# cschin/Peregrine

Hardware: AMD Instinct MI355X
Metric: confirmed overlaps/sec (ovlp_t records, index+overlap stages, seqdb resident in HBM) (higher is better)
Workload: dtype u8/u32 integer

## Files before the change

peregrine_amd/csrc/pgx_align.hip:

```cpp

#include "pgx_internal.h"

namespace pgx {
namespace {

__device__ __forceinline__ uint64_t load_u64_unaligned(const uint8_t *p) {
  uint64_t v;
  __builtin_memcpy(&v, p, 8);
  return v;
}
struct U128 {
  uint64_t lo, hi;
};
__device__ __forceinline__ U128 load_u128_unaligned(const uint8_t *p) {
  U128 v;
  __builtin_memcpy(&v, p, 16);
  return v;
}
__device__ __forceinline__ int match8(uint64_t qa, uint64_t ta, int qs, int ts) {
  const uint64_t diff = ((qa >> qs) ^ (ta >> ts)) & 0x0F0F0F0F0F0F0F0FULL;
  return diff ? (__builtin_ctzll(diff) >> 3) : 8;
}
__device__ __forceinline__ uint64_t ballot64(bool p) { return __builtin_amdgcn_ballot_w64(p); }
template <int CTRL>
__device__ __forceinline__ int dpp_max(int v) {
  return max(v, __builtin_amdgcn_update_dpp(0, v, CTRL, 0xf, 0xf, true));
}
template <int GL>
__device__ __forceinline__ int group_max_i32(int v) {
  static_assert(GL == 4 || GL == 8, "a group is a quad or half a DPP row");
  v = dpp_max<0xB1>(v);
  v = dpp_max<0x4E>(v);
  return GL == 8 ? dpp_max<0x141>(v) : v;
}
template <int GL>
__device__ __forceinline__ uint32_t group_bits(uint64_t wave_mask, int gbase) {
  return (uint32_t)(wave_mask >> gbase) & ((1u << GL) - 1u);
}
template <int CTRL>
__device__ __forceinline__ int dpp_min(int v) {
  return min(v, __builtin_amdgcn_update_dpp(0, v, CTRL, 0xf, 0xf, true));
}
template <int GL>
__device__ __forceinline__ int group_min_i32(int v) {
  v = dpp_min<0xB1>(v);
  v = dpp_min<0x4E>(v);
  return GL == 8 ? dpp_min<0x141>(v) : v;
}
__device__ __forceinline__ uint32_t ffbl_or_ones(uint32_t v) {
  uint32_t r;
  asm("v_ffbl_b32 %0, %1" : "=v"(r) : "v"(v));
  return r;
}
__device__ __forceinline__ int group_lane(int v, int gb4, int l) { return __builtin_amdgcn_ds_bpermute(gb4 + (l << 2), v); }

template <int CTRL, int ROW_MASK>
__device__ __forceinline__ int dpp_max_step(int v) {
  return max(v, __builtin_amdgcn_update_dpp(v, v, CTRL, ROW_MASK, 0xf, false));
}
__device__ __forceinline__ int wave_max_i32(int v) {
  v = dpp_max_step<0x111, 0xf>(v);
  v = dpp_max_step<0x112, 0xf>(v);
  v = dpp_max_step<0x114, 0xf>(v);
  v = dpp_max_step<0x118, 0xf>(v);
  v = dpp_max_step<0x142, 0xa>(v);
  v = dpp_max_step<0x143, 0xc>(v);
  return __builtin_amdgcn_readlane(v, 63);
}


}

__device__ __forceinline__ int match16p(const uint8_t *q, uint32_t xq, const uint8_t *t, uint32_t yt) {
  uint2 qd, td;
  __builtin_memcpy(&qd, q + (xq >> 4) * 4, 8), __builtin_memcpy(&td, t + (yt >> 4) * 4, 8);
  const uint32_t df = __builtin_amdgcn_alignbit(qd.y, qd.x, (xq & 15) << 1) ^ __builtin_amdgcn_alignbit(td.y, td.x, (yt & 15) << 1);
  return (int)min(ffbl_or_ones(df) >> 1, 16u);
}
__device__ __forceinline__ uint32_t target_offset(const pgx_align_key &) { return 0u; }
__device__ __forceinline__ uint32_t target_offset(const pgx_align_key2 &k) { return k.t_off; }
template <bool PACKED, typename KEY = pgx_align_key>
__device__ __forceinline__ void align_one_per_wave(const uint8_t *__restrict__ seq, const uint64_t *__restrict__ roff,
                                                   const uint32_t *__restrict__ rlen, const KEY *__restrict__ keys, uint32_t a, int band,
                                                   int ring, pgx_match *__restrict__ out) {
  static_assert(!PACKED || std::is_same_v<KEY, pgx_align_key>, "a target offset is honoured by the byte form only");
  extern __shared__ int32_t V[];
  constexpr int PB = PACKED ? 16 : 8;
  const int lane = threadIdx.x;
  const KEY key = keys[a];
  const uint32_t len0 = rlen[key.rid0], len1 = rlen[key.rid1];
  const uint8_t *q = PACKED ? seq + (roff[key.rid0] + (key.dir0 ? (len0 + 15u) >> 4 : 0u) + (key.q_off >> 4)) * 4 : seq + roff[key.rid0] + key.q_off;
  const uint8_t *t = PACKED ? seq + (roff[key.rid1] + (key.dir1 ? (len1 + 15u) >> 4 : 0u)) * 4 : seq + roff[key.rid1] + target_offset(key);
  const uint32_t qo = PACKED ? key.q_off & 15u : 0u;
  const int q_len = (int)(len0 - key.q_off);
  const int t_len = (int)(len1 - target_offset(key));
  const int qs = key.dir0 ? 4 : 0, ts = key.dir1 ? 4 : 0;
  const int max_d = (int)(0.3 * (double)(q_len + t_len));
  const int band_size = band * 2;
  const int mask = ring - 1;
  for (int i = lane; i < ring; i += 64) V[i] = 0;
  __syncthreads();

  int best_m = -1, min_k = 0, max_k = 0;
  uint32_t longest = 0;
  bool started = false, matched = false;
  int q_bgn = 0, t_bgn = 0, q_m_end = 0, t_m_end = 0, q_end = 0, t_end = 0, dist = 0;

  for (int d = 0; d < max_d; ++d) {
    if (max_k - min_k > band_size) break;
    const int nk = max_k >= min_k ? ((max_k - min_k) >> 1) + 1 : 0;
    int x = 0, y = 0;
    for (int base = 0; base < nk && !matched; base += 64) {
      const int j = base + lane;
      const bool active = j < nk;
      const int k = min_k + 2 * j;
      int x1 = 0, y1 = 0;
      x = 0, y = 0;
      bool more = false;
      if (active) {
        const int va = V[(k - 1) & mask], vb = V[(k + 1) & mask];
        x = (k == min_k || (k != max_k && va < vb)) ? vb : va + 1;
        y = x - k;
        x1 = x, y1 = y;
        const int rem = min(q_len - x, t_len - y);
        if (rem > 0) {
          int m = PACKED ? match16p(q, qo + (uint32_t)x, t, (uint32_t)y) : match8(load_u64_unaligned(q + x), load_u64_unaligned(t + y), qs, ts);
          m = min(m, rem);
          x += m, y += m;
          more = (m == PB) && (rem > PB);
        }
      }
      uint64_t mm = ballot64(more);
      while (mm) {
        const int L = __builtin_ctzll(mm);
        const int xs = __builtin_amdgcn_readlane(x, L), ys = __builtin_amdgcn_readlane(y, L);
        const int rem = min(q_len - xs, t_len - ys);
        const int off = lane * PB;
        int m = 0;
        if (off < rem)
          m = min(PACKED ? match16p(q, qo + (uint32_t)(xs + off), t, (uint32_t)(ys + off))
                         : match8(load_u64_unaligned(q + xs + off), load_u64_unaligned(t + ys + off), qs, ts), rem - off);
        const uint64_t stop = ballot64(m < PB);
        int ext;
        if (stop) {
          const int f = __builtin_ctzll(stop);
          ext = PB * f + __builtin_amdgcn_readlane(m, f);
        } else {
          ext = 64 * PB;
        }
        if (lane == L) x += ext, y += ext;
        if (stop || ext >= rem) mm &= mm - 1;
      }
      const int ext = x - x1;
      const bool hit = active && (x >= q_len || y >= t_len);
      const uint64_t hitmask = ballot64(hit);
      const int hl = hitmask ? __builtin_ctzll(hitmask) : 64;
      const bool valid = active && lane <= hl;
      if (!started) {
        const uint64_t m = ballot64(valid && ext > 16);
        if (m) {
          const int l = __builtin_ctzll(m);
          q_bgn = __builtin_amdgcn_readlane(x1, l), t_bgn = __builtin_amdgcn_readlane(y1, l);
          started = true;
        }
      }
      if (ballot64(valid && (uint32_t)ext > longest)) {
        const int mx = wave_max_i32(valid ? ext : -1);
        const int l = __builtin_ctzll(ballot64(valid && ext == mx));
        longest = (uint32_t)mx;
        q_m_end = __builtin_amdgcn_readlane(x, l), t_m_end = __builtin_amdgcn_readlane(y, l);
      }
      if (valid) V[k & mask] = x;
      best_m = max(best_m, wave_max_i32(valid ? x + y : -1));
      if (hitmask) {
        matched = true;
        q_end = __builtin_amdgcn_readlane(x, hl), t_end = __builtin_amdgcn_readlane(y, hl);
      }
    }
    __syncthreads();
    if (matched) {
      dist = d;
      break;
    }
    int new_min = max_k, new_max = min_k;
    const int thr = best_m - band;
    for (int base = 0; base < nk; base += 64) {
      const int j = base + lane;
      const int k2 = min_k + 2 * j;
      int u;
      if (nk <= 64) u = x + y;
      else u = j < nk ? 2 * V[k2 & mask] - k2 : 0;
      const uint64_t m = ballot64(j < nk && u >= thr);
      if (m) {
        new_min = min(new_min, min_k + 2 * (base + __builtin_ctzll(m)));
        new_max = max(new_max, min_k + 2 * (base + 63 - __builtin_clzll(m)));
      }
    }
    max_k = new_max + 1;
    min_k = new_min - 1;
  }
  if (lane == 0) {
    pgx_match r;
    if (matched) {
      r.q_bgn = q_bgn, r.t_bgn = t_bgn, r.q_end = q_end, r.t_end = t_end, r.dist = dist;
      r.m_size = (q_end - q_bgn + t_end - t_bgn + 2 * dist) / 2;
    } else {
      r.q_bgn = 0, r.t_bgn = 0, r.q_end = 0, r.t_end = 0, r.dist = 0, r.m_size = 0;
    }
    r.q_m_end = q_m_end, r.t_m_end = t_m_end;
    out[a] = r;
  }
}
template <bool PACKED>
__global__ __launch_bounds__(64) void k_align1(const uint8_t *__restrict__ seq, const uint64_t *__restrict__ roff,
                                              const uint32_t *__restrict__ rlen,
                                              const pgx_align_key *__restrict__ keys, uint32_t n, int band,
                                              int ring, pgx_match *__restrict__ out) {
  if (blockIdx.x < n) align_one_per_wave<PACKED>(seq, roff, rlen, keys, blockIdx.x, band, ring, out);
}
__global__ __launch_bounds__(64) void k_align1t(const uint8_t *__restrict__ seq, const uint64_t *__restrict__ roff, const uint32_t *__restrict__ rlen,
                                               const pgx_align_key2 *__restrict__ keys, uint32_t n, int band, int ring, pgx_match *__restrict__ out) {
  if (blockIdx.x < n) align_one_per_wave<false, pgx_align_key2>(seq, roff, rlen, keys, blockIdx.x, band, ring, out);
}
__global__ __launch_bounds__(64) void k_align1_handon(const uint8_t *__restrict__ seq, const uint64_t *__restrict__ roff,
                                                     const uint32_t *__restrict__ rlen, const pgx_align_key *__restrict__ keys, uint32_t n, int band,
                                                     int ring, pgx_match *__restrict__ out, const uint32_t *__restrict__ nflag,
                                                     uint32_t *__restrict__ hand_n, uint32_t *__restrict__ hand_list) {
  if (blockIdx.x >= n) return;
  const pgx_align_key key = keys[blockIdx.x];
  if ((nflag[key.rid0] | nflag[key.rid1]) & 1u) {
    if (threadIdx.x == 0) hand_list[atomicAdd(hand_n, 1u)] = blockIdx.x;
    return;
  }
  align_one_per_wave<true>(seq, roff, rlen, keys, blockIdx.x, band, ring, out);
}
template <bool PACKED>
__global__ __launch_bounds__(64) void k_align1_list(const uint8_t *__restrict__ seq, const uint64_t *__restrict__ roff,
                                                   const uint32_t *__restrict__ rlen, const pgx_align_key *__restrict__ keys,
                                                   const uint32_t *__restrict__ list_n, const uint32_t *__restrict__ list, int band, int ring,
                                                   pgx_match *__restrict__ out) {
  const uint32_t cnt = *list_n;
  for (uint32_t i = blockIdx.x; i < cnt; i += gridDim.x) {
    __syncthreads();
    align_one_per_wave<PACKED>(seq, roff, rlen, keys, list[i], band, ring, out);
  }
}


enum { PH_FETCH = 0, PH_STEP = 1, PH_ROUND = 2, PH_SNAKE = 3, PH_END = 4, PH_BAND = 5, PH_DONE = 6 };
#define PH_SYNC() __builtin_amdgcn_fence(__ATOMIC_RELEASE, "wavefront"), __builtin_amdgcn_fence(__ATOMIC_ACQUIRE, "wavefront")
template <typename VT, bool PACKED, int GL>
__global__ __launch_bounds__(1024, 8) void k_align_ph(const uint8_t *__restrict__ seq, const uint64_t *__restrict__ roff,
                                                      const uint32_t *__restrict__ rlen, const pgx_align_key *__restrict__ keys,
                                                      uint32_t n, int band, int ring, pgx_match *__restrict__ out,
                                                      uint32_t *__restrict__ counter, const uint32_t *__restrict__ redo_n,
                                                      const uint32_t *__restrict__ redo_list, uint32_t *__restrict__ esc_n,
                                                      uint32_t *__restrict__ esc_list, const uint32_t *__restrict__ nflag, uint32_t seg,
                                                      uint32_t iter_limit) {
  extern __shared__ int32_t Vall[];
  __shared__ unsigned long long s_state;
  __shared__ uint32_t s_lock;
  const int lane = threadIdx.x & 63, gl = lane & (GL - 1), gbase = lane & ~(GL - 1), gb4 = gbase << 2;
  VT *V = reinterpret_cast<VT *>(Vall) + ((threadIdx.x >> 6) * (64 / GL) + lane / GL) * ring;
  if (threadIdx.x == 0) s_state = (unsigned long long)seg, s_lock = 0u;
  __syncthreads();
  const int mask2 = (ring - 1) << 1, band_size = band * 2;
  const auto slot = [&](int kd) -> VT & {
    return *reinterpret_cast<VT *>(reinterpret_cast<char *>(V) + (kd & mask2) * (int)(sizeof(VT) / 2));
  };
  constexpr int SL = PACKED ? 32 : 16;
  constexpr int PROBE = PACKED ? 16 : 8;
  if (redo_list) n = *redo_n;
  const uint32_t iter_budget = esc_list && iter_limit ? iter_limit : 0xFFFFFFFFu;
  uint32_t qo = 0, to = 0;
  uint32_t iters = 0;
  uint32_t c_next = 0, c_end = 0;

  int phase = PH_FETCH;
  uint32_t a = 0;
  const uint8_t *q = seq, *t = seq;
  int q_len = 0, t_len = 0, qs = 0, ts = 0, max_d = 0, d = 0;
  int best_m = -1, min_k = 0, max_k = 0, nk = 0, base = 0, bbase = 0, new_min = 0, new_max = 0;
  uint32_t longest = 0;
  bool started = false;
  int q_bgn = 0, t_bgn = 0, q_m_end = 0, t_m_end = 0;
  int x = 0, y = 0, x1 = 0, y1 = 0, k = 0;
  bool active = false;
  uint32_t gm = 0;

#ifdef PGX_ALIGN_STATS
  uint32_t my_iters = 0;
  int my_maxnk = 0;
  bool has_cand = false;
  const bool stats_on = !redo_list || redo_n == esc_n + 3;
#endif
  for (;;) {
#ifdef PGX_ALIGN_STATS
    if (phase == PH_FETCH && has_cand && gl == 0 && stats_on) {
      const uint32_t b = my_iters ? 31u - (uint32_t)__builtin_clz(my_iters) : 0u;
      atomicAdd(counter + 1 + min(b, 31u), 1u);
#ifdef PGX_ALIGN_STATS_NK
      atomicAdd(counter + 33 + min((uint32_t)my_maxnk, 31u), 1u);
#else
      atomicAdd(counter + 33 + min(b, 31u), my_iters);
#endif
    }
    if (phase == PH_FETCH) has_cand = false, my_iters = 0, my_maxnk = 0;
    my_maxnk = max(my_maxnk, phase == PH_ROUND || phase == PH_STEP ? nk : 0);
    ++my_iters;
#endif
    ++iters;
    constexpr uint32_t RETRY = 0xFFFFFFFFu;
    const bool fetching = phase == PH_FETCH;
    const uint64_t fw = ballot64(fetching);
    uint32_t na = 0;
    if (fw) {
      constexpr uint32_t CHUNK = 64 / GL;
      const uint64_t need = fw & (GL == 8 ? 0x0101010101010101ULL : 0x1111111111111111ULL);
      const uint32_t cnt = (uint32_t)__builtin_popcountll(need);
      const uint32_t r = __builtin_amdgcn_mbcnt_hi((uint32_t)(need >> 32), __builtin_amdgcn_mbcnt_lo((uint32_t)need, 0u));
      const uint32_t avail = __builtin_amdgcn_readfirstlane(c_end - c_next);
      na = c_next + r;
      if (avail < cnt) {
        uint32_t got = RETRY;
        if (lane == 0) {
          unsigned long long o = atomicAdd(&s_state, (unsigned long long)CHUNK);
          if ((uint32_t)o < seg) {
            got = (uint32_t)(o >> 32) + (uint32_t)o;
          } else if (atomicCAS(&s_lock, 0u, 1u) == 0u) {
            o = atomicAdd(&s_state, (unsigned long long)CHUNK);
            if ((uint32_t)o < seg) {
              got = (uint32_t)(o >> 32) + (uint32_t)o;
            } else {
              got = atomicAdd(counter, seg);
              atomicExch(&s_state, ((unsigned long long)got << 32) | CHUNK);
            }
            atomicExch(&s_lock, 0u);
          }
        }
        got = __builtin_amdgcn_readfirstlane(got);
        if (got == RETRY) {
          if (r >= avail) na = RETRY;
          c_next = c_end = 0;
        } else {
          if (r >= avail) na = got + (r - avail);
          c_next = got + (cnt - avail), c_end = got + CHUNK;
        }
      } else {
        c_next += cnt;
      }
    }
    if (fetching) {
      iters = 0;
      na = (uint32_t)group_lane((int)na, gb4, 0);
      if (na == RETRY) {
      } else if (na >= n) {
        phase = PH_DONE;
      } else {
#ifdef PGX_ALIGN_STATS
        has_cand = true;
#endif
        a = redo_list ? redo_list[na] : na;
        const pgx_align_key key = keys[a];
        const uint32_t len0 = rlen[key.rid0], len1 = rlen[key.rid1];
        if (PACKED) {
          q = seq + (roff[key.rid0] + (key.dir0 ? (len0 + 15u) >> 4 : 0u) + (key.q_off >> 4)) * 4;
          t = seq + (roff[key.rid1] + (key.dir1 ? (len1 + 15u) >> 4 : 0u)) * 4;
          qo = key.q_off & 15u, to = 0;
        } else {
          q = seq + roff[key.rid0] + key.q_off;
          t = seq + roff[key.rid1];
        }
        q_len = (int)(len0 - key.q_off);
        t_len = (int)len1;
        qs = key.dir0 ? 4 : 0, ts = key.dir1 ? 4 : 0;
        max_d = (int)(0.3 * (double)(q_len + t_len));
        d = 0, best_m = -1, min_k = 0, max_k = 0, longest = 0;
        started = false;
        q_bgn = t_bgn = q_m_end = t_m_end = 0;
        if (gl == 0) slot(2) = (VT)0;
        phase = PH_STEP;
        if (PACKED && ((nflag[key.rid0] | nflag[key.rid1]) & 1u)) {
          if (gl == 0) esc_list[n + atomicAdd(esc_n + 1, 1u)] = a;
          phase = PH_FETCH;
        }
      }
    }
    if (!ballot64(phase != PH_DONE)) break;
    PH_SYNC();

    if (iters > iter_budget && phase == PH_STEP && !(d >= max_d || max_k - min_k > band_size)) {
      if (gl == 0) esc_list[atomicAdd(esc_n, 1u)] = a;
      phase = PH_FETCH;
    }
    if (phase == PH_STEP) {
      const int width = max_k - min_k;
      if (d >= max_d || width > band_size) {
        if (gl == 0) {
          pgx_match r;
          r.m_size = 0, r.dist = 0, r.q_bgn = 0, r.q_end = 0, r.t_bgn = 0, r.t_end = 0;
          r.t_m_end = t_m_end, r.q_m_end = q_m_end;
          out[a] = r;
        }
        phase = PH_FETCH;
      } else if (width < 0) {
        nk = 0, base = 0, bbase = 0, new_min = max_k, new_max = min_k, phase = PH_BAND;
      } else {
        nk = (width >> 1) + 1, base = 0, phase = PH_ROUND;
      }
    }

    int probe_full = 0;
    if (phase == PH_ROUND) {
      const int j = base + gl;
      active = j < nk;
      k = min_k + 2 * j;
      if (active) {
        const int va = (int)slot(k - d), vb = (int)slot(k - d + 2);
        x = (k == min_k || (k != max_k && va < vb)) ? vb : va + 1;
        y = x - k;
        x1 = x, y1 = y;
        const int rem = min(q_len - x, t_len - y);
        if (rem > 0) {
          int m;
          if (PACKED) {
            const uint32_t xq = qo + (uint32_t)x, yt = to + (uint32_t)y;
            uint2 qd, td;
            __builtin_memcpy(&qd, q + (xq >> 4) * 4, 8), __builtin_memcpy(&td, t + (yt >> 4) * 4, 8);
            const uint32_t df = __builtin_amdgcn_alignbit(qd.y, qd.x, (xq & 15) << 1) ^ __builtin_amdgcn_alignbit(td.y, td.x, (yt & 15) << 1);
            m = (int)min(ffbl_or_ones(df) >> 1, 16u);
          } else {
            m = match8(load_u64_unaligned(q + x), load_u64_unaligned(t + y), qs, ts);
          }
          probe_full = (int)min((uint32_t)m, (uint32_t)(rem - 1));
          m = (int)min((uint32_t)m, (uint32_t)rem);
          x += m, y += m;
        }
      }
    }
    {
      asm volatile("" : "+v"(probe_full));
      const uint32_t g = group_bits<GL>(ballot64(probe_full >= PROBE), gbase);
      if (phase == PH_ROUND) gm = g, phase = g ? PH_SNAKE : PH_END;
    }

    {
      const bool sn = phase == PH_SNAKE;
      if (ballot64(sn)) {
        const int L = __builtin_ctz(gm | (1u << GL));
        const int xs = group_lane(x, gb4, L), ys = group_lane(y, gb4, L);
        const int rem = min(q_len - xs, t_len - ys);
        const int off = gl * SL;
        int e = GL * SL;
        if (sn) {
          e = off;
          if (off < rem) {
            int m;
            if (PACKED) {
              const uint32_t xq = qo + (uint32_t)(xs + off), yt = to + (uint32_t)(ys + off);
              uint4 qd, td;
              __builtin_memcpy(&qd, q + (xq >> 4) * 4, 16), __builtin_memcpy(&td, t + (yt >> 4) * 4, 16);
              const uint32_t qsh = (xq & 15) << 1, tsh = (yt & 15) << 1;
              const uint32_t d0 = __builtin_amdgcn_alignbit(qd.y, qd.x, qsh) ^ __builtin_amdgcn_alignbit(td.y, td.x, tsh);
              const uint32_t d1 = __builtin_amdgcn_alignbit(qd.z, qd.y, qsh) ^ __builtin_amdgcn_alignbit(td.z, td.y, tsh);
              m = (int)min(min(ffbl_or_ones(d0), ffbl_or_ones(d1) | 32u) >> 1, 32u);
            } else {
              const U128 qa = load_u128_unaligned(q + xs + off), ta = load_u128_unaligned(t + ys + off);
              m = match8(qa.lo, ta.lo, qs, ts);
              if (m == 8) m += match8(qa.hi, ta.hi, qs, ts);
            }
            m = (int)min((uint32_t)m, (uint32_t)(rem - off));
            e = m < SL ? off + m : GL * SL;
          }
        }
        const int ext = group_min_i32<GL>(e);
        if (sn) {
          if (gl == L) x += ext, y += ext;
          if (ext < GL * SL || ext >= rem) gm &= gm - 1;
          if (!gm) phase = PH_END;
        }
      }
    }

    {
      const bool e = phase == PH_END;
      const int ext = x - x1;
      const bool hit = e && active && (x >= q_len || y >= t_len);
      const uint64_t hitw = ballot64(hit);
      int hl = GL;
      uint32_t hitm = 0;
      if (hitw) {
        hitm = group_bits<GL>(hitw, gbase);
        if (hitm) hl = __builtin_ctz(hitm);
        asm volatile("" : "+v"(hl));
      }
      const bool valid = e && active && gl <= hl;
      {
        const uint64_t sw = ballot64((valid && !started ? ext : 0) > 16);
        if (sw) {
          const uint32_t m = group_bits<GL>(sw, gbase);
          const int l = m ? __builtin_ctz(m) : 0;
          const int bx = group_lane(x1, gb4, l), by = group_lane(y1, gb4, l);
          if (m) q_bgn = bx, t_bgn = by, started = true;
        }
      }
      const int ev = valid ? ext : -1;
      if (ballot64(ev > (int)longest)) {
        const int mx = group_max_i32<GL>(ev);
        const uint32_t m = group_bits<GL>(ballot64(valid && ext == mx), gbase);
        const int l = m ? __builtin_ctz(m) : 0;
        const int ex = group_lane(x, gb4, l), ey = group_lane(y, gb4, l);
        if (e && mx >= 0 && (uint32_t)mx > longest) longest = (uint32_t)mx, q_m_end = ex, t_m_end = ey;
      }
      if (valid) slot(k - d) = (VT)x;
      const int u = x + y;
      {
        const int s = group_max_i32<GL>(valid ? u : -1);
        if (e) best_m = max(best_m, s);
      }
      bool matched = false;
      if (hitw) {
        const int ex = group_lane(x, gb4, hl & (GL - 1)), ey = group_lane(y, gb4, hl & (GL - 1));
        if (e && hitm) {
          matched = true;
          if (gl == 0) {
            pgx_match r;
            r.q_bgn = q_bgn, r.t_bgn = t_bgn, r.q_end = ex, r.t_end = ey, r.dist = d;
            r.m_size = (ex - q_bgn + ey - t_bgn + 2 * d) / 2;
            r.t_m_end = t_m_end, r.q_m_end = q_m_end;
            out[a] = r;
          }
        }
      }
      const uint32_t qm = group_bits<GL>(ballot64((e && active ? u : INT32_MIN) >= best_m - band), gbase);
      const bool wide_step = e && !matched && nk > GL;
      if (ballot64(wide_step)) {
        const bool last = wide_step && base + GL >= nk;
        if (wide_step) {
          if (base == 0) new_min = max_k, new_max = min_k;
          if (qm) {
            new_min = min(new_min, min_k + 2 * (base + __builtin_ctz(qm)));
            new_max = max(new_max, min_k + 2 * (base + 31 - __builtin_clz(qm)));
          }
          base += GL;
          phase = PH_ROUND;
        }
        if (ballot64(last)) {
          const bool some = last && new_min <= new_max;
          const int ke = gl ? new_max : new_min;
          int ue = INT32_MIN;
          if (some && gl < 2) ue = 2 * (int)slot(ke - d) - ke;
          const uint32_t pm = group_bits<GL>(ballot64(ue >= best_m - band), gbase);
          if (last) {
            if (!some || (pm & 3u) == 3u) {
              max_k = new_max + 1, min_k = new_min - 1, ++d, phase = PH_STEP;
            } else {
              bbase = 0, new_min = max_k, new_max = min_k, phase = PH_BAND;
            }
#ifdef PGX_ALIGN_STATS
            if (gl == 0 && stats_on) atomicAdd(counter + (phase == PH_BAND ? 66 : 65), 1u);
#endif
          }
        }
      }
      if (e && !wide_step) {
        if (matched) {
          phase = PH_FETCH;
        } else {
          const int lo = qm ? min_k + 2 * __builtin_ctz(qm) : max_k, hi = qm ? min_k + 2 * (31 - __builtin_clz(qm)) : min_k;
          max_k = hi + 1, min_k = lo - 1, ++d, phase = PH_STEP;
        }
      }
    }
    PH_SYNC();

    {
      const bool bnd = phase == PH_BAND;
      if (ballot64(bnd)) {
        const int thr = best_m - band;
        const int j = bbase + gl;
        const int k2 = min_k + 2 * j;
        int u = 0;
        if (bnd && j < nk) u = 2 * (int)slot(k2 - d) - k2;
        const uint32_t m = group_bits<GL>(ballot64((bnd && j < nk ? u : INT32_MIN) >= thr), gbase);
        if (bnd) {
          if (m) {
            new_min = min(new_min, min_k + 2 * (bbase + __builtin_ctz(m)));
            new_max = max(new_max, min_k + 2 * (bbase + 31 - __builtin_clz(m)));
          }
          bbase += GL;
          if (bbase >= nk) max_k = new_max + 1, min_k = new_min - 1, ++d, phase = PH_STEP;
        }
      }
    }
  }
}

__global__ void k_order_keys(const pgx_align_key *__restrict__ keys, uint32_t n, const uint32_t *__restrict__ prank, uint32_t *__restrict__ k,
                             uint32_t *__restrict__ v, uint32_t *__restrict__ n_out) {
  const uint32_t i = blockIdx.x * blockDim.x + threadIdx.x;
  if (i == 0) *n_out = n;
  if (i < n) k[i] = prank[keys[i].rid0], v[i] = i;
}

struct SeqSource {
  const uint8_t *seq;
  const uint64_t *off;
  bool packed;
};
static SeqSource seq_bytes(const pgx_seqdb *db) { return {db->d_seq.p, db->d_roff.p, false}; }
static SeqSource seq_packed(const pgx_seqdb *db) { return {reinterpret_cast<const uint8_t *>(db->d_pack.p), db->d_poff.p, true}; }
struct AlignSources {
  SeqSource grouped;
  SeqSource one;
  bool compacted;
};
static AlignSources align_source(const pgx_seqdb *db, long grouped_n) {
  if (seq_compacted(db)) {
    PGX_REQUIRE(seq_packs_valid(db), PGX_ESTATE, "the seqdb's bytes were compacted (pgx_seqdb_compact_bytes) and its packs are gone");
    return {seq_packed(db), seq_packed(db), true};
  }
  const bool has_bytes = db->d_seq.p != nullptr, short_reads = db->max_rlen <= 65535u;
  const char *p1 = getenv("PGX_ALIGN1_PACKED");
  const bool one_packed = seq_packs_valid(db) && db->n_flagged_reads == 0 && short_reads && (!has_bytes || !(p1 && atoi(p1) == 0));
  const char *pm = getenv("PGX_ALIGN_PACKED_MIN");
  const long packed_min = pm ? atol(pm) : 100000;
  const bool grouped_packed = short_reads && grouped_n >= 0 &&
                              (!has_bytes || (packed_min >= 0 && (grouped_n >= packed_min || seq_packs_valid(db)))) && seq_packs(db) != nullptr;
  PGX_REQUIRE(has_bytes || (one_packed && (grouped_n < 0 || grouped_packed)), PGX_ESTATE,
              "the seqdb's bytes were released (pgx_seqdb_release_bytes) and its packs are gone");
  return {grouped_packed ? seq_packed(db) : seq_bytes(db), one_packed ? seq_packed(db) : seq_bytes(db), false};
}
template <typename K, typename... A>
void launch_on(const SeqSource &s, K on_packs, K on_bytes, dim3 grid, dim3 block, size_t lds, A... args) {
  hipLaunchKernelGGL(s.packed ? on_packs : on_bytes, grid, block, lds, ctx().stream, s.seq, s.off, args...);
}

void dev_align_prepare(const pgx_seqdb *db) { (void)align_source(db, LONG_MAX); }

void dev_align(const pgx_seqdb *db, const pgx_align_key *d_keys, size_t n, int band, pgx_match *d_out, int tail_batch) {
  if (n == 0) return;
  const long small_max = getenv("PGX_ALIGN_SMALL") ? atol(getenv("PGX_ALIGN_SMALL")) : tail_batch >= 2 ? 250000 : tail_batch ? 60000 : 13000;
  const bool small = (long)n <= small_max;
  KernelTimer tm(small ? "align1" : "align", n);
  int ring = 64;
  while (ring < 2 * band + 8) ring <<= 1;
  hipStream_t st = ctx().stream;
  const AlignSources src = align_source(db, small ? -1 : (long)n);
  if (small && src.compacted) {
    uint32_t *hand = ws<uint32_t>("align.handon", n + 4);
    PGX_HIP(hipMemsetAsync(hand, 0, sizeof(uint32_t), st));
    hipLaunchKernelGGL(k_align1_handon, dim3((unsigned)n), dim3(64), ring * sizeof(int32_t), st, src.one.seq, src.one.off, db->d_rlen.p, d_keys, (uint32_t)n,
                       band, ring, d_out, db->d_nflag.p, hand, hand + 4);
    PGX_HIP(hipGetLastError());
    uint32_t nh = 0;
    PGX_HIP(hipMemcpyAsync(&nh, hand, sizeof(uint32_t), hipMemcpyDeviceToHost, st));
    sync();
    if (nh) {
      ByteView view;
      side_view_of_keys(db, d_keys, hand + 4, nh, view);
      hipLaunchKernelGGL(k_align1_list<false>, dim3(std::min<unsigned>(nh, (unsigned)ctx().num_cu * 32)), dim3(64), ring * sizeof(int32_t), st, view.seq,
                         view.off, db->d_rlen.p, d_keys, hand, hand + 4, band, ring, d_out);
      PGX_HIP(hipGetLastError());
    }
    return;
  }
  if (small) {
    launch_on(src.one, k_align1<true>, k_align1<false>, dim3((unsigned)n), dim3(64), ring * sizeof(int32_t), db->d_rlen.p, d_keys, (uint32_t)n, band,
              ring, d_out);
    PGX_HIP(hipGetLastError());
    return;
  }
#ifdef PGX_ALIGN_STATS
  constexpr size_t n_counter = 72;
#else
  constexpr size_t n_counter = 8;
#endif
  uint32_t *counter = ws<uint32_t>("align.counter", n_counter);
  PGX_HIP(hipMemsetAsync(counter, 0, n_counter * sizeof(uint32_t), st));
  const bool wide = db->max_rlen > 65535u;
  const long gl_env = getenv("PGX_ALIGN_GL") ? atol(getenv("PGX_ALIGN_GL")) : 0;
  const int gl = wide ? 8 : (gl_env == 4 || gl_env == 8) ? (int)gl_env : (src.grouped.packed && tail_batch == 0) ? 4 : 8;
  const size_t chunk = 64 / gl;
  int ring_ph = 32;
  while (ring_ph < band + 2) ring_ph <<= 1;
  const size_t lds_wave = chunk * ring_ph * (wide ? sizeof(int32_t) : sizeof(uint16_t));
  const unsigned waves_cu = (unsigned)std::min<size_t>(32, (158u << 10) / lds_wave);
  const long nw_env = getenv("PGX_ALIGN_NW") ? atol(getenv("PGX_ALIGN_NW")) : 0;
  unsigned NW = 1;
  for (unsigned c = 16; c >= 1; c >>= 1)
    if (c <= waves_cu && (waves_cu / c) * c > (waves_cu / NW) * NW) NW = c;
  if (waves_cu >= 16 && (waves_cu / 16) * 16 >= (waves_cu / NW) * NW) NW = 16;
  if (nw_env >= 1 && nw_env <= 16 && (unsigned)nw_env <= waves_cu) NW = (unsigned)nw_env;
  const size_t lds = lds_wave * NW;
  const unsigned wg_cu = waves_cu / NW;
  const size_t n_wg = (size_t)ctx().num_cu * wg_cu;
  auto segment = [&](size_t cnt) {
    const long se = getenv("PGX_ALIGN_SEG") ? atol(getenv("PGX_ALIGN_SEG")) : 0;
    size_t sg = se > 0 ? (size_t)se : std::min<size_t>(64 * chunk, std::max<size_t>(chunk * NW, cnt / (n_wg * 16)));
    return (uint32_t)((sg + chunk - 1) & ~(chunk - 1));
  };
  const uint32_t seg = segment(n);
  const unsigned grid = (unsigned)std::min<size_t>((n + seg - 1) / seg, n_wg);
  uint32_t *esc = nullptr;
  const uint32_t *order = nullptr;
  uint32_t iter_limit = 0;
  if (src.grouped.packed) {
    iter_limit = getenv("PGX_ALIGN_ITER_LIMIT") ? (uint32_t)atol(getenv("PGX_ALIGN_ITER_LIMIT")) : 2500u;
    esc = ws<uint32_t>("align.esc", 2 * n + 4);
    PGX_HIP(hipMemsetAsync(esc, 0, 3 * sizeof(uint32_t), st));
    const long order_min = getenv("PGX_ALIGN_ORDER_MIN") ? atol(getenv("PGX_ALIGN_ORDER_MIN")) : 200000;
    if (db->locus_ordered && order_min >= 0 && (long)n >= order_min) {
      const uint32_t nn = (uint32_t)n;
      uint32_t *k_in = ws<uint32_t>("align.ord_kin", n), *k_out = ws<uint32_t>("align.ord_kout", n), *v_in = ws<uint32_t>("align.ord_vin", n),
               *v_out = ws<uint32_t>("align.ord_vout", n);
      hipLaunchKernelGGL(k_order_keys, dim3((nn + 255) / 256), dim3(256), 0, st, d_keys, nn, db->d_prank.p, k_in, v_in, esc + 3);
      int bits = 1;
      while (bits < 32 && (db->rlen_by_rid.size() >> bits)) ++bits;
      sort_pairs(k_in, k_out, v_in, v_out, nn, 0, bits);
      order = v_out;
    }
  }
  const auto ph_bytes = wide ? k_align_ph<int32_t, false, 8> : gl == 4 ? k_align_ph<uint16_t, false, 4> : k_align_ph<uint16_t, false, 8>;
  const auto ph_packs = gl == 4 ? k_align_ph<uint16_t, true, 4> : k_align_ph<uint16_t, true, 8>;
  launch_on(src.grouped, ph_packs, ph_bytes, dim3(grid), dim3(64 * NW), lds, db->d_rlen.p, d_keys, (uint32_t)n, band, ring_ph, d_out,
            counter, order ? esc + 3 : nullptr, order, esc, esc ? esc + 4 : nullptr, db->d_nflag.p, seg, iter_limit);
#ifdef PGX_ALIGN_STATS
  {
    uint32_t h[n_counter];
    PGX_HIP(hipMemcpyAsync(h, counter, sizeof(h), hipMemcpyDeviceToHost, st));
    sync();
    unsigned long long cand = 0, total = 0;
    for (int b = 0; b < 32; ++b) cand += h[1 + b], total += h[33 + b];
    fprintf(stderr, "[pgx] align stats: %llu candidates, %llu wavefront iterations of theirs (tail_batch %d); per candidate (log2 classes: count, share of all iterations):",
            cand, total, tail_batch);
    for (int b = 0; b < 32; ++b)
      if (h[1 + b]) fprintf(stderr, " 2^%d: %u (%.1f %%)", b, h[1 + b], total ? 100.0 * h[33 + b] / (double)total : 0.0);
    fprintf(stderr, "; wide steps settled in END %u, sent to BAND %u\n", h[65], h[66]);
  }
#endif
  if (esc) {
    if (src.compacted) {
      uint32_t nf = 0;
      PGX_HIP(hipMemcpyAsync(&nf, esc + 1, sizeof(uint32_t), hipMemcpyDeviceToHost, st));
      sync();
      if (nf) {
        ByteView view;
        side_view_of_keys(db, d_keys, esc + 4 + n, nf, view);
        uint32_t *esc2 = ws<uint32_t>("align.esc_view", (size_t)nf + 4);
        PGX_HIP(hipMemsetAsync(esc2, 0, sizeof(uint32_t), st));
        hipLaunchKernelGGL(ph_bytes, dim3((unsigned)std::min<size_t>(nf / (64 * NW) + 8, n_wg)), dim3(64 * NW), lds, st, view.seq, view.off,
                           db->d_rlen.p, d_keys, (uint32_t)n, band, ring_ph, d_out, esc + 2, esc + 1, esc + 4 + n, esc2, esc2 + 4, (const uint32_t *)nullptr,
                           segment(nf / 16 + 1), iter_limit);
        hipLaunchKernelGGL(k_align1_list<false>, dim3(std::min<unsigned>(nf, (unsigned)ctx().num_cu * 32)), dim3(64), ring * sizeof(int32_t), st, view.seq,
                           view.off, db->d_rlen.p, d_keys, esc2, esc2 + 4, band, ring, d_out);
      }
    } else if (db->n_flagged_reads)
      launch_on(seq_bytes(db), ph_packs, ph_bytes, dim3((unsigned)std::min<size_t>(n / (64 * NW) + 8, n_wg)), dim3(64 * NW), lds,
                db->d_rlen.p, d_keys, (uint32_t)n, band, ring_ph, d_out, esc + 2, esc + 1, esc + 4 + n, esc, esc + 4, nullptr, segment(n / 16 + 1),
                iter_limit);
    const dim3 g1((unsigned)std::min<size_t>(std::max<size_t>(n / 256, 256), (size_t)ctx().num_cu * 32));
    launch_on(src.one, k_align1_list<true>, k_align1_list<false>, g1, dim3(64), ring * sizeof(int32_t), db->d_rlen.p, d_keys, esc, esc + 4, band,
              ring, d_out);
  }
  PGX_HIP(hipGetLastError());
}

void dev_align2(const pgx_seqdb *db, const uint8_t *seq, const uint64_t *off, const pgx_align_key2 *d_keys, size_t n, int band, pgx_match *d_out) {
  if (n == 0) return;
  KernelTimer tm("align1t", n);
  int ring = 64;
  while (ring < 2 * band + 8) ring <<= 1;
  hipLaunchKernelGGL(k_align1t, dim3((unsigned)n), dim3(64), ring * sizeof(int32_t), ctx().stream, seq, off, db->d_rlen.p, d_keys, (uint32_t)n, band, ring,
                     d_out);
  PGX_HIP(hipGetLastError());
}

}
```

Baseline: 71.34 million.

## Hand off escaped alignments with saved wavefront state to resume in one-per-wave kernel

When the grouped phase kernel exceeds its iteration budget (or an optional width budget), it now writes its diagonal index, band bounds, best-match state and the current V ring slots to a device arena before queuing the candidate for the one-wave-per-alignment fallback. The fallback kernel restores that state into LDS and continues from that diagonal, so it no longer restarts the alignment from scratch. A width-based hand-off knob (off by default) and extra stats counters are added. The cost is arena memory, extra global writes at hand-off, and more parameters per launch.

After: 70.34 million. 1.4% lower.

```diff
diff --git a/peregrine_amd/csrc/pgx_align.hip b/peregrine_amd/csrc/pgx_align.hip
--- a/peregrine_amd/csrc/pgx_align.hip
+++ b/peregrine_amd/csrc/pgx_align.hip
@@ -79,10 +79,12 @@
 }
 __device__ __forceinline__ uint32_t target_offset(const pgx_align_key &) { return 0u; }
 __device__ __forceinline__ uint32_t target_offset(const pgx_align_key2 &k) { return k.t_off; }
+constexpr int HANDON_HDR = 10;
+__host__ __device__ constexpr uint32_t handon_stride(int ring_ph) { return (uint32_t)(HANDON_HDR + ring_ph / 2); }
 template <bool PACKED, typename KEY = pgx_align_key>
 __device__ __forceinline__ void align_one_per_wave(const uint8_t *__restrict__ seq, const uint64_t *__restrict__ roff,
                                                    const uint32_t *__restrict__ rlen, const KEY *__restrict__ keys, uint32_t a, int band,
-                                                   int ring, pgx_match *__restrict__ out) {
+                                                   int ring, pgx_match *__restrict__ out, const uint32_t *__restrict__ rec = nullptr) {
   static_assert(!PACKED || std::is_same_v<KEY, pgx_align_key>, "a target offset is honoured by the byte form only");
   extern __shared__ int32_t V[];
   constexpr int PB = PACKED ? 16 : 8;
@@ -105,8 +107,17 @@
   uint32_t longest = 0;
   bool started = false, matched = false;
   int q_bgn = 0, t_bgn = 0, q_m_end = 0, t_m_end = 0, q_end = 0, t_end = 0, dist = 0;
-
-  for (int d = 0; d < max_d; ++d) {
+  int d0 = 0;
+  if (rec) {
+    d0 = (int)rec[0], min_k = (int)rec[1], max_k = (int)rec[2], best_m = (int)rec[3], longest = rec[4], started = rec[5] != 0u;
+    q_bgn = (int)rec[6], t_bgn = (int)rec[7], q_m_end = (int)rec[8], t_m_end = (int)rec[9];
+    const uint16_t *sl = reinterpret_cast<const uint16_t *>(rec + HANDON_HDR);
+    const int nslots = max_k >= min_k ? ((max_k - min_k) >> 1) + 2 : 0;
+    for (int j = lane; j < nslots; j += 64) V[(min_k - 1 + 2 * j) & mask] = (int32_t)sl[j];
+    __syncthreads();
+  }
+
+  for (int d = d0; d < max_d; ++d) {
     if (max_k - min_k > band_size) break;
     const int nk = max_k >= min_k ? ((max_k - min_k) >> 1) + 1 : 0;
     int x = 0, y = 0;
@@ -238,16 +249,17 @@
 __global__ __launch_bounds__(64) void k_align1_list(const uint8_t *__restrict__ seq, const uint64_t *__restrict__ roff,
                                                    const uint32_t *__restrict__ rlen, const pgx_align_key *__restrict__ keys,
                                                    const uint32_t *__restrict__ list_n, const uint32_t *__restrict__ list, int band, int ring,
-                                                   pgx_match *__restrict__ out) {
+                                                   pgx_match *__restrict__ out, const uint32_t *__restrict__ arena, uint32_t arena_cap,
+                                                   uint32_t arena_stride) {
   const uint32_t cnt = *list_n;
   for (uint32_t i = blockIdx.x; i < cnt; i += gridDim.x) {
     __syncthreads();
-    align_one_per_wave<PACKED>(seq, roff, rlen, keys, list[i], band, ring, out);
-  }
-}
-
-
-enum { PH_FETCH = 0, PH_STEP = 1, PH_ROUND = 2, PH_SNAKE = 3, PH_END = 4, PH_BAND = 5, PH_DONE = 6 };
+    align_one_per_wave<PACKED>(seq, roff, rlen, keys, list[i], band, ring, out, i < arena_cap ? arena + (size_t)i * arena_stride : nullptr);
+  }
+}
+
+
+enum { PH_FETCH = 0, PH_STEP = 1, PH_ROUND = 2, PH_SNAKE = 3, PH_END = 4, PH_BAND = 5, PH_DONE = 6, PH_HANDON = 7 };
 #define PH_SYNC() __builtin_amdgcn_fence(__ATOMIC_RELEASE, "wavefront"), __builtin_amdgcn_fence(__ATOMIC_ACQUIRE, "wavefront")
 template <typename VT, bool PACKED, int GL>
 __global__ __launch_bounds__(1024, 8) void k_align_ph(const uint8_t *__restrict__ seq, const uint64_t *__restrict__ roff,
@@ -256,7 +268,8 @@
                                                       uint32_t *__restrict__ counter, const uint32_t *__restrict__ redo_n,
                                                       const uint32_t *__restrict__ redo_list, uint32_t *__restrict__ esc_n,
                                                       uint32_t *__restrict__ esc_list, const uint32_t *__restrict__ nflag, uint32_t seg,
-                                                      uint32_t iter_limit) {
+                                                      uint32_t iter_limit, uint32_t handon_nk, uint32_t *__restrict__ arena,
+                                                      uint32_t arena_cap) {
   extern __shared__ int32_t Vall[];
   __shared__ unsigned long long s_state;
   __shared__ uint32_t s_lock;
@@ -272,6 +285,7 @@
   constexpr int PROBE = PACKED ? 16 : 8;
   if (redo_list) n = *redo_n;
   const uint32_t iter_budget = esc_list && iter_limit ? iter_limit : 0xFFFFFFFFu;
+  const int nk_budget = esc_list && handon_nk ? (int)min(handon_nk, 0x7FFFFFFFu) : 0x7FFFFFFF;
   uint32_t qo = 0, to = 0;
   uint32_t iters = 0;
   uint32_t c_next = 0, c_end = 0;
@@ -291,6 +305,7 @@
 #ifdef PGX_ALIGN_STATS
   uint32_t my_iters = 0;
   int my_maxnk = 0;
+  uint32_t my_wide[4] = {0, 0, 0, 0};
   bool has_cand = false;
   const bool stats_on = !redo_list || redo_n == esc_n + 3;
 #endif
@@ -304,8 +319,11 @@
 #else
       atomicAdd(counter + 33 + min(b, 31u), my_iters);
 #endif
-    }
-    if (phase == PH_FETCH) has_cand = false, my_iters = 0, my_maxnk = 0;
+      for (int w = 0; w < 4; ++w)
+        if (my_wide[w]) atomicAdd(counter + 70 + w, my_wide[w]);
+      atomicAdd(counter + 74, my_iters);
+    }
+    if (phase == PH_FETCH) has_cand = false, my_iters = 0, my_maxnk = 0, my_wide[0] = my_wide[1] = my_wide[2] = my_wide[3] = 0;
     my_maxnk = max(my_maxnk, phase == PH_ROUND || phase == PH_STEP ? nk : 0);
     ++my_iters;
 #endif
@@ -389,10 +407,6 @@
     if (!ballot64(phase != PH_DONE)) break;
     PH_SYNC();
 
-    if (iters > iter_budget && phase == PH_STEP && !(d >= max_d || max_k - min_k > band_size)) {
-      if (gl == 0) esc_list[atomicAdd(esc_n, 1u)] = a;
-      phase = PH_FETCH;
-    }
     if (phase == PH_STEP) {
       const int width = max_k - min_k;
       if (d >= max_d || width > band_size) {
@@ -408,7 +422,38 @@
       } else {
         nk = (width >> 1) + 1, base = 0, phase = PH_ROUND;
       }
-    }
+      if (phase != PH_FETCH && (iters > iter_budget || nk > nk_budget)) phase = PH_HANDON;
+    }
+    if (phase == PH_HANDON) {
+      x = y = x1 = y1 = k = 0, base = bbase = new_min = new_max = 0, gm = 0, active = false;
+      uint32_t pos = 0;
+      if (gl == 0) {
+        pos = atomicAdd(esc_n, 1u);
+        esc_list[pos] = a;
+#ifdef PGX_ALIGN_STATS
+        if (stats_on) atomicAdd(counter + (iters > iter_budget ? 67 : 68), 1u), atomicAdd(counter + 69, pos < arena_cap && sizeof(VT) == 2 ? 0u : 1u);
+#endif
+      }
+      pos = (uint32_t)group_lane((int)pos, gb4, 0);
+      if (sizeof(VT) == 2 && pos < arena_cap) {
+        char *rec = reinterpret_cast<char *>(arena) + pos * (handon_stride(ring) * 4u);
+        const auto word = [&](int i) -> uint32_t & { return *reinterpret_cast<uint32_t *>(rec + 4 * i); };
+        if (gl == 0) {
+          word(0) = (uint32_t)d, word(1) = (uint32_t)min_k, word(2) = (uint32_t)max_k, word(3) = (uint32_t)best_m, word(4) = longest;
+          word(5) = started ? 1u : 0u, word(6) = (uint32_t)q_bgn, word(7) = (uint32_t)t_bgn, word(8) = (uint32_t)q_m_end, word(9) = (uint32_t)t_m_end;
+        }
+        int j0 = gl;
+        asm volatile("" : "+v"(j0));
+#pragma clang loop unroll(disable) vectorize(disable)
+        for (int j = j0; j <= nk; j += GL)
+          *reinterpret_cast<uint16_t *>(rec + 4 * HANDON_HDR + 2 * j) = (uint16_t)slot(min_k - d + 2 * j);
+      }
+      phase = PH_FETCH;
+    }
+#ifdef PGX_ALIGN_STATS
+    if (phase == PH_ROUND || phase == PH_SNAKE || phase == PH_BAND)
+      for (int w = 0; w < 4; ++w) my_wide[w] += nk > (8 << w) ? 1u : 0u;
+#endif
 
     int probe_full = 0;
     if (phase == PH_ROUND) {
@@ -603,6 +648,16 @@
   if (i < n) k[i] = prank[keys[i].rid0], v[i] = i;
 }
 
+constexpr uint32_t HANDON_NK_MAIN = 0, HANDON_NK_TAIL = 0, ITER_LIMIT = 2500;
+static uint32_t launch_knob(const char *name, int tail_batch, uint32_t dflt) {
+  const char *e = getenv(name);
+  if (!e) return dflt;
+  char *end = nullptr;
+  long v = strtol(e, &end, 10);
+  if (tail_batch && end && *end == ',') v = strtol(end + 1, nullptr, 10);
+  return (uint32_t)std::max(0L, v);
+}
+
 struct SeqSource {
   const uint8_t *seq;
   const uint64_t *off;
@@ -660,7 +715,7 @@
       ByteView view;
       side_view_of_keys(db, d_keys, hand + 4, nh, view);
       hipLaunchKernelGGL(k_align1_list<false>, dim3(std::min<unsigned>(nh, (unsigned)ctx().num_cu * 32)), dim3(64), ring * sizeof(int32_t), st, view.seq,
-                         view.off, db->d_rlen.p, d_keys, hand, hand + 4, band, ring, d_out);
+                         view.off, db->d_rlen.p, d_keys, hand, hand + 4, band, ring, d_out, (const uint32_t *)nullptr, 0u, 0u);
       PGX_HIP(hipGetLastError());
     }
     return;
@@ -672,7 +727,7 @@
     return;
   }
 #ifdef PGX_ALIGN_STATS
-  constexpr size_t n_counter = 72;
+  constexpr size_t n_counter = 80;
 #else
   constexpr size_t n_counter = 8;
 #endif
@@ -704,9 +759,17 @@
   const unsigned grid = (unsigned)std::min<size_t>((n + seg - 1) / seg, n_wg);
   uint32_t *esc = nullptr;
   const uint32_t *order = nullptr;
-  uint32_t iter_limit = 0;
+  uint32_t iter_limit = 0, handon_nk = 0, arena_cap = 0;
+  uint32_t *arena = nullptr;
   if (src.grouped.packed) {
-    iter_limit = getenv("PGX_ALIGN_ITER_LIMIT") ? (uint32_t)atol(getenv("PGX_ALIGN_ITER_LIMIT")) : 2500u;
+    iter_limit = launch_knob("PGX_ALIGN_ITER_LIMIT", tail_batch, ITER_LIMIT);
+    if (!wide && !src.compacted) {
+      const size_t cap = getenv("PGX_ALIGN_ARENA_CAP") ? (size_t)std::max(0L, atol(getenv("PGX_ALIGN_ARENA_CAP")))
+                                                       : std::max<size_t>(n / 64, 65536);
+      arena_cap = (uint32_t)std::min(std::min(cap, n), (size_t)0xFFFF0000u / (handon_stride(ring_ph) * 4u));
+      if (arena_cap) arena = ws<uint32_t>("align.handon_arena", (size_t)arena_cap * handon_stride(ring_ph));
+    }
+    handon_nk = launch_knob("PGX_ALIGN_HANDON_NK", tail_batch, !arena_cap ? 0u : tail_batch ? HANDON_NK_TAIL : HANDON_NK_MAIN);
     esc = ws<uint32_t>("align.esc", 2 * n + 4);
     PGX_HIP(hipMemsetAsync(esc, 0, 3 * sizeof(uint32_t), st));
     const long order_min = getenv("PGX_ALIGN_ORDER_MIN") ? atol(getenv("PGX_ALIGN_ORDER_MIN")) : 200000;
@@ -724,7 +787,7 @@
   const auto ph_bytes = wide ? k_align_ph<int32_t, false, 8> : gl == 4 ? k_align_ph<uint16_t, false, 4> : k_align_ph<uint16_t, false, 8>;
   const auto ph_packs = gl == 4 ? k_align_ph<uint16_t, true, 4> : k_align_ph<uint16_t, true, 8>;
   launch_on(src.grouped, ph_packs, ph_bytes, dim3(grid), dim3(64 * NW), lds, db->d_rlen.p, d_keys, (uint32_t)n, band, ring_ph, d_out,
-            counter, order ? esc + 3 : nullptr, order, esc, esc ? esc + 4 : nullptr, db->d_nflag.p, seg, iter_limit);
+            counter, order ? esc + 3 : nullptr, order, esc, esc ? esc + 4 : nullptr, db->d_nflag.p, seg, iter_limit, handon_nk, arena, arena_cap);
 #ifdef PGX_ALIGN_STATS
   {
     uint32_t h[n_counter];
@@ -736,7 +799,9 @@
             cand, total, tail_batch);
     for (int b = 0; b < 32; ++b)
       if (h[1 + b]) fprintf(stderr, " 2^%d: %u (%.1f %%)", b, h[1 + b], total ? 100.0 * h[33 + b] / (double)total : 0.0);
-    fprintf(stderr, "; wide steps settled in END %u, sent to BAND %u\n", h[65], h[66]);
+    fprintf(stderr, "; wide steps settled in END %u, sent to BAND %u", h[65], h[66]);
+    fprintf(stderr, "; handed on by budget %u, by width %u, of them without a record %u; iterations %u, of them in steps of nk > 8: %u, > 16: %u, > 32: %u, > 64: %u\n",
+            h[67], h[68], h[69], h[74], h[70], h[71], h[72], h[73]);
   }
 #endif
   if (esc) {
@@ -751,17 +816,17 @@
         PGX_HIP(hipMemsetAsync(esc2, 0, sizeof(uint32_t), st));
         hipLaunchKernelGGL(ph_bytes, dim3((unsigned)std::min<size_t>(nf / (64 * NW) + 8, n_wg)), dim3(64 * NW), lds, st, view.seq, view.off,
                            db->d_rlen.p, d_keys, (uint32_t)n, band, ring_ph, d_out, esc + 2, esc + 1, esc + 4 + n, esc2, esc2 + 4, (const uint32_t *)nullptr,
-                           segment(nf / 16 + 1), iter_limit);
+                           segment(nf / 16 + 1), iter_limit, handon_nk, (uint32_t *)nullptr, 0u);
         hipLaunchKernelGGL(k_align1_list<false>, dim3(std::min<unsigned>(nf, (unsigned)ctx().num_cu * 32)), dim3(64), ring * sizeof(int32_t), st, view.seq,
-                           view.off, db->d_rlen.p, d_keys, esc2, esc2 + 4, band, ring, d_out);
+                           view.off, db->d_rlen.p, d_keys, esc2, esc2 + 4, band, ring, d_out, (const uint32_t *)nullptr, 0u, 0u);
       }
     } else if (db->n_flagged_reads)
       launch_on(seq_bytes(db), ph_packs, ph_bytes, dim3((unsigned)std::min<size_t>(n / (64 * NW) + 8, n_wg)), dim3(64 * NW), lds,
                 db->d_rlen.p, d_keys, (uint32_t)n, band, ring_ph, d_out, esc + 2, esc + 1, esc + 4 + n, esc, esc + 4, nullptr, segment(n / 16 + 1),
-                iter_limit);
-    const dim3 g1((unsigned)std::min<size_t>(std::max<size_t>(n / 256, 256), (size_t)ctx().num_cu * 32));
+                iter_limit, handon_nk, arena, arena_cap);
+    const dim3 g1((unsigned)std::min<size_t>(std::max<size_t>(n / (handon_nk ? 16 : 256), 256), (size_t)ctx().num_cu * 32));
     launch_on(src.one, k_align1_list<true>, k_align1_list<false>, g1, dim3(64), ring * sizeof(int32_t), db->d_rlen.p, d_keys, esc, esc + 4, band,
-              ring, d_out);
+              ring, d_out, (const uint32_t *)arena, arena_cap, handon_stride(ring_ph));
   }
   PGX_HIP(hipGetLastError());
 }
```
